# GREAT-WHU/DBA-Fusion

Hardware: AMD Instinct MI355X
Metric: DBA iterations/sec (25-KF, 96-edge, 512x512) [dba_update/s] (higher is better)
Workload: dtype f32 (BA, f64 reduced system) / f16 (correlation)

## Files before the change

dba-fusion_amd/csrc/ba_host.hip:

```cpp
#include <hip/hip_runtime.h>

#include <algorithm>
#include <atomic>
#include <cstdio>
#include <cstdlib>
#include <cstring>
#include <mutex>
#include <unordered_map>
#include <vector>

#include "ba_kernels.h"

#ifndef GRAM_F32_DEFAULT
#define GRAM_F32_DEFAULT true
#endif

namespace dba {

static thread_local char g_last_error[512] = "";

void set_last_error(const char *what, hipError_t e) {
  snprintf(g_last_error, sizeof(g_last_error), "%s -> %s", what, hipGetErrorString(e));
}

struct BaEnv {
  static int num(const char *name) { const char *e = getenv(name); return e ? atoi(e) : 0; }
  static bool is(const char *name, const char *prefix) { const char *e = getenv(name); return e && !strncmp(e, prefix, strlen(prefix)); }
  int deterministic = is("DBA_DETERMINISTIC", "1");
  int solve_check = is("DBA_SOLVE_CHECK", "1");
  int schur_form = is("DBA_SCHUR_KERNEL", "r") ? 1 : (is("DBA_SCHUR_KERNEL", "f") || is("DBA_SCHUR_KERNEL", "g")) ? 2 : 0;
  int lin_ppl = num("DBA_LINEARIZE_PPL");
  bool lin_no_mfma = is("DBA_LINEARIZE_MFMA", "0");
  int lin_ew = num("DBA_LIN_EW");
  bool h_full = is("DBA_H_FULL", "1");
  int schur_nch = num("DBA_SCHUR_NCH");
  int gram_threads = num("DBA_SCHUR_WAVES") == 4 ? 256 : 512;
  bool gram_f32 = getenv("DBA_SCHUR_MFMA") ? is("DBA_SCHUR_MFMA", "f3") : GRAM_F32_DEFAULT;
  bool fuse_update = !is("DBA_BA_FUSE_UPDATE", "0");
};
static const BaEnv &ba_env() { static const BaEnv env; return env; }

static std::atomic<int> g_schur_form{ba_env().schur_form};
static std::atomic<int> g_deterministic{ba_env().deterministic};
static std::atomic<int> g_solve_check{ba_env().solve_check};

__global__ __launch_bounds__(256) void ba_solve_check_kernel(const double *__restrict__ H, const double *__restrict__ b, int n, double lm,
                                                             double ep, float *__restrict__ dx, int *__restrict__ meta) {
  __shared__ double s_res[256], s_mag[256];
  __shared__ int s_bad;
  if (meta[1] != 0) return;
  double res = 0.0, mag = 0.0;
  for (int i = threadIdx.x; i < n; i += blockDim.x) {
    double acc = -b[i], m = fabs(b[i]);
    for (int j = 0; j < n; j++) {
      double h = H[(size_t)max(i, j) * n + min(i, j)];
      if (i == j) h = fma(lm, h, h) + ep;
      const double t = h * (double)dx[j];
      acc += t, m += fabs(t);
    }
    res = fmax(res, fabs(acc)), mag = fmax(mag, m);
  }
  s_res[threadIdx.x] = res, s_mag[threadIdx.x] = mag;
  __syncthreads();
  if (threadIdx.x == 0) {
    double r = 0.0, m = 0.0;
    for (int k = 0; k < (int)blockDim.x; k++) r = fmax(r, s_res[k]), m = fmax(m, s_mag[k]);
    s_bad = !(r <= 1e-5 * m) ? 1 : 0;
    if (s_bad) meta[1] = 1;
  }
  __syncthreads();
  if (s_bad)
    for (int i = threadIdx.x; i < n; i += blockDim.x) dx[i] = 0.f;
}

static bool schur_auto_frame_form(int N, int P) {
  const int frames = P + 1;
  const int rows_est = 1 + (N + frames - 1) / frames;
  return rows_est > 6;
}

static std::atomic<int> g_schur_generation{0};
static thread_local int t_schur_form = 0;

bool ba_schur_frame_form(int N, int P) {
  const int forced = g_schur_form.load(std::memory_order_relaxed);
  if (N + 1 > GRAM_LIST_CAP) return false;
  if (forced) return forced == 2;
  if (t_schur_form) return t_schur_form == 2;
  return schur_auto_frame_form(N, P);
}

// ... 64 lines not shown
    plan->T.meta = reinterpret_cast<int *>(base + L.meta);
    plan->T.kx = reinterpret_cast<int *>(base + L.kx);
    plan->T.frame_slot = reinterpret_cast<int *>(base + o_fslot);
    plan->T.eoff = reinterpret_cast<int *>(base + o_eoff);
    plan->T.elist = reinterpret_cast<int *>(base + o_elist);
    plan->T.elist_rank = reinterpret_cast<int *>(base + o_erank);
    plan->T.fpose = reinterpret_cast<int *>(base + o_fpose);
    plan->T.einfo = reinterpret_cast<int *>(base + o_einfo);
    plan->T.rowinfo = reinterpret_cast<int *>(base + o_rowinfo);
    plan->T.fhead = reinterpret_cast<int *>(base + o_fhead);
    plan->T.frow = reinterpret_cast<int *>(base + o_frow);
    plan->T.gkey = reinterpret_cast<int *>(base + o_gkey);
    plan->T.Mmax = Mmax;
    plan->T.B = B;
    plan->W.E = reinterpret_cast<float *>(base + L.E);
    plan->W.Q = reinterpret_cast<float *>(base + L.Q);
    plan->W.w = reinterpret_cast<float *>(base + L.w);
    plan->W.HpartE = reinterpret_cast<float *>(base + o_hparte);
    plan->W.Aedge = reinterpret_cast<double *>(base + o_aedge);
    plan->W.dx = reinterpret_cast<float *>(base + L.dx);
    plan->W.poses_tmp = reinterpret_cast<float *>(base + o_ptmp);
    plan->W.H = reinterpret_cast<double *>(base + L.H);
    plan->W.b = reinterpret_cast<double *>(base + L.b);
    plan->W.Lscratch = want_scratch ? reinterpret_cast<double *>(base + o_lscratch) : nullptr;
    plan->W.nparts = nparts;
    plan->W.ppl = ppl;
  }
  return DBA_OK;
}

static int ba_prepare_stage(const BaPlan &plan, const int64_t *ii, const int64_t *jj, int eta_rows, int check, bool judge_band,
                            hipStream_t stream) {
  const int N = plan.N, B = plan.B, P = plan.P;
  if (N > 0 && (!ii || !jj)) return DBA_ERR_ARG;
  const int want = std::max(std::max(N, B), P);
  const int threads = std::min(1024, std::max(64, (want + 63) / 64 * 64));
  const size_t scan_ints = std::max<size_t>(std::max(threads, P), N > threads ? 1024 : 0) + 32;
  const size_t lds = sizeof(int) * ((size_t)B + 2 * (size_t)plan.T.Mmax + 1 + scan_ints + plan.T.Mmax + 1);
  if (lds > 160 * 1024 || P > 16384) return DBA_ERR_UNSUPPORTED;
  if (lds > 64 * 1024) {
    DBA_HIP_CHECK(hipFuncSetAttribute(reinterpret_cast<const void *>(&ba_prepare_kernel),
                                      hipFuncAttributeMaxDynamicSharedMemorySize, 160 * 1024));
  }
  const int max_nt = judge_band ? ba_solve_wave_max_nt(6 * P) : 0;
  int *band_verdict = max_nt ? solver_verdict_slot(plan.T.meta) : nullptr;
  hipLaunchKernelGGL(ba_prepare_kernel, dim3(1), dim3(threads), lds, stream, ii, jj, N, B, plan.t0, plan.t1,
                     (int)scan_ints, ba_schur_frame_form(N, P) ? 1 : 0, check ? 1 : 0, eta_rows,
                     eta_rows > 1 ? ws_eta_status(plan.T.meta) : nullptr, plan.T, band_verdict, max_nt);
  DBA_LAUNCH_CHECK();
  return DBA_OK;
}

static int ba_linearize_stage(const BaPlan &plan, const BaProblem &g, const float *poses, const float *disps, float alpha,
                              int upd, float *poses_out, float *disps_w, hipStream_t stream) {
  if (!poses || !disps || !g.intrinsics || !g.disps_sens || !g.eta || g.eta_rows < 1) return DBA_ERR_ARG;
  if (g.eta_rows > 1 && g.eta_rows > plan.T.Mmax) return DBA_ERR_ARG;
  if (plan.N > 0 && (!g.targets || !g.weights || !g.jj)) return DBA_ERR_ARG;
#define LAUNCH_LIN(PPL, MF, EW)                                                                                          \
  hipLaunchKernelGGL((ba_linearize_kernel<PPL, MF, EW>), dim3(plan.nchunks * EW, plan.T.Mmax + 1), dim3(256), 0, stream, \
                     poses, disps, g.intrinsics, g.disps_sens, g.targets, g.weights, g.eta, g.eta_rows, g.jj,            \
                     g.frame_owned, plan.N, plan.HW, plan.wd, plan.t0, plan.P, alpha, upd, poses_out, disps_w, plan.T, plan.W)
  if (plan.W.ppl == 4) LAUNCH_LIN(4, false, 1);
  else if (plan.W.ppl == 2) LAUNCH_LIN(2, false, 1);
  else if (ba_env().lin_no_mfma) LAUNCH_LIN(1, false, 1);
  else {
    const int env_ew = ba_env().lin_ew;
    const long waves2 = (long)plan.nchunks * 2 * 4 * plan.T.Mmax;
    const bool one = env_ew ? env_ew == 1 : waves2 > 4096;
    if (one) LAUNCH_LIN(1, true, 1);
    else LAUNCH_LIN(1, true, 2);
  }
#undef LAUNCH_LIN
  DBA_LAUNCH_CHECK();
  return DBA_OK;
}

static int ba_reduce_stage(const BaPlan &plan, const int64_t *ii, const int64_t *jj, const uint8_t *frame_owned, int motion_only,
                           int lower, hipStream_t stream) {
  const int N = plan.N;
  const int ablocks = (N + 3) / 4;
  if (plan.P <= 0) return DBA_OK;
  if (ba_env().h_full) lower = 0;
  const bool fixed = g_deterministic.load(std::memory_order_relaxed) != 0;
  if (fixed) lower |= 2;
  if (!motion_only) {
    if (!ba_schur_frame_form(N, plan.P)) {
      hipLaunchKernelGGL(ba_schur_kernel, dim3(plan.P + N + ablocks, SCHUR_KP, SCHUR_CH), dim3(256), 0, stream, ii, jj,
                         frame_owned, N, plan.HW, plan.t0, plan.P, lower, plan.T, plan.W);
    } else {
      const int px = 1024;
      int nch = ba_env().schur_nch > 0 ? ba_env().schur_nch : (plan.HW + px - 1) / px;
      nch = std::max(1, std::min(nch, (plan.HW + 15) / 16));
      const dim3 grid((unsigned)(plan.T.Mmax * nch + ablocks));
      const int gram_threads = ba_env().gram_threads;
      const bool f32 = ba_env().gram_f32;
#define GRAM_LAUNCH(V, F)                                                                                     \
  hipLaunchKernelGGL((ba_schur_gram_kernel<V, F>), grid, dim3(gram_threads), 0, stream, ii, jj, frame_owned, \
                     N, plan.HW, plan.t0, plan.P, nch, lower, plan.T, plan.W)
      if (plan.HW % 4 == 0) { if (f32) GRAM_LAUNCH(true, true); else GRAM_LAUNCH(true, false); }
      else { if (f32) GRAM_LAUNCH(false, true); else GRAM_LAUNCH(false, false); }
#undef GRAM_LAUNCH
    }
    DBA_LAUNCH_CHECK();
  } else if (ablocks > 0) {
    hipLaunchKernelGGL(ba_assemble_kernel, dim3(ablocks), dim3(256), 0, stream, ii, jj, frame_owned, N, plan.t0, plan.P,
                       lower, plan.T, plan.W);
    DBA_LAUNCH_CHECK();
  }
  if (fixed) {
    const int n = 6 * plan.P;
    hipLaunchKernelGGL(ba_fixed_to_f64_kernel, dim3((n * n + n + 255) / 256), dim3(256), 0, stream, plan.W.H, plan.W.b, n);
    DBA_LAUNCH_CHECK();
  }
  return DBA_OK;
}

static int ba_symmetrize_launch(const BaPlan &plan, hipStream_t stream) {
  const int n = 6 * plan.P;
  if (n <= 0) return DBA_OK;
  hipLaunchKernelGGL(ba_symmetrize_kernel, dim3((n * n + 255) / 256), dim3(256), 0, stream, plan.W.H, n);
  DBA_LAUNCH_CHECK();
  return DBA_OK;
}

static int ba_solve_check_launch(const BaPlan &plan, float lm, float ep, hipStream_t stream) {
  if (plan.P <= 0) return DBA_OK;
  hipLaunchKernelGGL(ba_solve_check_kernel, dim3(1), dim3(256), 0, stream, plan.W.H, plan.W.b, 6 * plan.P, (double)lm, (double)ep,
                     plan.W.dx, plan.T.meta);
  DBA_LAUNCH_CHECK();
  return DBA_OK;
}

static int ba_solve_stage(const BaPlan &plan, float lm, float ep, const int *fpose, int hint, hipStream_t stream) {
  const int rc = launch_ba_solve(plan.W.H, plan.W.b, fpose, 6 * plan.P, (double)lm, (double)ep, plan.W.dx, plan.T.meta,
                                 plan.W.Lscratch, stream, nullptr, hint, (fpose && fpose == plan.T.fpose) ? plan.T.meta + 16 : nullptr);
  if (rc != DBA_OK) return rc;
  if (g_solve_check.load(std::memory_order_relaxed)) return ba_solve_check_launch(plan, lm, ep, stream);
  return DBA_OK;
}

static int ba_update_launch(const BaPlan &plan, float *poses, float *disps, const int64_t *jj, const uint8_t *frame_owned,
                            int update_poses, int update_disps, float *dz_out, float *dx_out, hipStream_t stream,
                            const float *poses_src = nullptr, float disp_floor = 0.f) {
  dim3 grid((plan.HW + 255) / 256, plan.T.Mmax + 1 + (disp_floor > 0.f ? plan.B : 0));
  hipLaunchKernelGGL(ba_update_kernel, grid, dim3(256), 0, stream, poses, poses_src, disps, jj, frame_owned, plan.HW, plan.t0,
                     plan.P, update_poses, update_disps, dz_out, dx_out, plan.T, plan.W, disp_floor);
  DBA_LAUNCH_CHECK();
  return DBA_OK;
}

int ba_run_loop(const BaPlan &plan, const BaProblem &g, float *poses, float *disps, const BaRun &run, hipStream_t stream) {
  const int *fpose = run.window_fpose ? run.window_fpose : plan.T.fpose;
  int rc;
  if (run.prepared != 1) {
    rc = ba_prepare_stage(plan, g.ii, g.jj, g.eta_rows, run.prepared == 2, run.window_fpose == nullptr, stream);
    if (rc != DBA_OK) return rc;
  }
  const bool fuse = ba_env().fuse_update;
  const float *pose_src = poses;
  bool pending = false;
  for (int itr = 0; itr < run.iterations; itr++) {
    float *pose_dst = plan.W.poses_tmp + (size_t)(itr & 1) * 7 * plan.B;
    const int upd = pending ? (run.motion_only ? 1 : 3) : 0;
    rc = ba_linearize_stage(plan, g, pose_src, disps, run.alpha, upd, pending ? pose_dst : nullptr, disps, stream);
    if (rc != DBA_OK) return rc;
    if (pending) pose_src = pose_dst;
    rc = ba_reduce_stage(plan, g.ii, g.jj, g.frame_owned, run.motion_only, 1, stream);
    if (rc != DBA_OK) return rc;
    if (run.exchange && run.exchange->fn && plan.P > 0) {
      const size_t n6 = (size_t)6 * plan.P;
      rc = run.exchange->fn(run.exchange->ctx, plan.W.H, (size_t)(plan.W.b - plan.W.H) + n6, stream);
      if (rc != DBA_OK) return rc;
    }
    rc = ba_solve_stage(plan, run.lm, run.ep, fpose, run.solver_hint, stream);
    if (rc != DBA_OK) return rc;
    const bool last = (itr == run.iterations - 1);
    if (fuse && !last) {
      pending = true;
      continue;
    }
    rc = ba_update_launch(plan, poses, disps, g.jj, g.frame_owned, 1, run.motion_only ? 0 : 1, last ? run.dz_out : nullptr,
                          last ? run.dx_out : nullptr, stream, pose_src == poses ? nullptr : pose_src,
                          last ? run.disp_floor : 0.f);
    if (rc != DBA_OK) return rc;
    pose_src = poses;
    pending = false;
  }
  return DBA_OK;
}

namespace {
struct BacoreStage {
  double *host = nullptr;
  size_t doubles = 0;
  unsigned *counter = nullptr;
  int seq = 0;
};
std::mutex g_stage_mu;
typedef std::unordered_map<const void *, BacoreStage> BacoreStageMap;
BacoreStageMap *stage_map_ptr() {
  static BacoreStageMap *m = new BacoreStageMap;
  return m;
}
#define stage_map() (*stage_map_ptr())
int *stage_flag(const BacoreStage &st) { return reinterpret_cast<int *>(st.host + st.doubles + 8); }
}

static int bacore_stage_for(const int *meta, size_t need, hipStream_t stream, BacoreStage **out) {
  std::lock_guard<std::mutex> lock(g_stage_mu);
  BacoreStage &st = stage_map()[meta];
  if (st.doubles < need) {
    if (st.host) {
      DBA_HIP_CHECK(hipStreamSynchronize(stream));
      (void)hipHostFree(st.host);
      st.host = nullptr, st.doubles = 0;
    }
    void *p = nullptr;
// ... 388 lines not shown
```

dba-fusion_amd/csrc/ba_kernels.h:

```cpp
#pragma once
#include "common.h"

namespace dba {

constexpr int HPE_STRIDE = 32;
#ifndef SCHUR_KP_CFG
#define SCHUR_KP_CFG 8
#endif
#ifndef SCHUR_CH_CFG
#define SCHUR_CH_CFG 2
#endif
constexpr int SCHUR_KP = SCHUR_KP_CFG;
constexpr int SCHUR_CH = SCHUR_CH_CFG;

struct BaTables {
  int *meta;
  int *kx;
  int *frame_slot;
  int *eoff;
  int *elist;
  int *elist_rank;
  int *fpose;
  int *einfo;
  int *rowinfo;
  int *fhead;
  int *frow;
  int *gkey;
  int Mmax, B;
};

struct BaBuffers {
  float *E;
  float *Q;
  float *w;
  float *HpartE;
  double *Aedge;
  double *H;
  double *b;
  float *dx;
  double *Lscratch;
  float *poses_tmp;
  int nparts;
  int ppl;
};

struct BaPlan {
  BaTables T;
  BaBuffers W;
  dba_ba_layout layout;
  size_t bytes;
  int P, N, B, HW, nchunks;
  int ht, wd, t0, t1;
};

int ba_plan(int N, int B, int ht, int wd, int t0, int t1, void *ws, size_t ws_bytes, BaPlan *plan);
#define DBA_PLAN_OR_RETURN(plan) \
  BaPlan plan;                   \
  if (const int plan_rc_ = ::dba::ba_plan(N, B, ht, wd, t0, t1, ws, ws_bytes, &plan)) return plan_rc_

constexpr int GKEY_MAGIC = 0x6b657935;
__global__ void ba_prepare_kernel(const int64_t *ii, const int64_t *jj, int N, int B, int t0, int t1, int scan_ints,
                                  int ftable, int check, int eta_rows, int *status, BaTables T, int *band_verdict, int max_nt);
bool ba_schur_frame_form(int N, int P);
template <int PPL, bool MF, int EW>
__global__ void ba_linearize_kernel(const float *poses, const float *disps, const float *intrinsics,
                                    const float *disps_sens, const float *targets, const float *weights,
                                    const float *eta, int eta_rows, const int64_t *jj,
                                    const uint8_t *frame_owned, int N, int HW, int wd, int t0, int P,
                                    float alpha, int upd, float *poses_out, float *disps_w, BaTables T, BaBuffers W);
__global__ void ba_assemble_kernel(const int64_t *ii, const int64_t *jj, const uint8_t *frame_owned, int N,
                                   int t0, int P, int lower, BaTables T, BaBuffers W);
__global__ void ba_schur_kernel(const int64_t *ii, const int64_t *jj, const uint8_t *frame_owned, int N, int HW,
                                int t0, int P, int lower, BaTables T, BaBuffers W);
__global__ void ba_symmetrize_kernel(double *H, int n);
struct ExportArg {
  double A[36];
};
__global__ void ba_export_kernel(const double *H, const double *b, int n, double *out, int gtsam, ExportArg arg, double stab,
                                 unsigned *counter, int *host_flag, int seq);
__global__ void ba_fixed_to_f64_kernel(double *H, double *b, int n);
constexpr int GRAM_LIST_CAP = 1024;
template <bool VEC, bool F32>
__global__ void ba_schur_gram_kernel(const int64_t *ii, const int64_t *jj, const uint8_t *frame_owned, int N, int HW,
                                     int t0, int P, int nch, int lower, BaTables T, BaBuffers W);
__global__ void ba_update_kernel(float *poses, const float *poses_src, float *disps, const int64_t *jj, const uint8_t *frame_owned,
                                 int HW, int t0, int P, int update_poses, int update_disps, float *dz_out,
                                 float *dx_out, BaTables T, BaBuffers W, float disp_floor);
__global__ void ba_copy_f32_kernel(const float *src, float *dst, int n);
__global__ void ba_gather_edges_kernel(const float2 *tgt_inac, const float2 *wgt_inac, const int64_t *ii_inac, const int64_t *jj_inac,
                                       const int64_t *sel, int n_sel, int n_inac, const float2 *tgt_act, const float2 *wgt_act,
                                       const int64_t *ii_act, const int64_t *jj_act, int HW, float *tgt_out, float *wgt_out,
                                       int64_t *ii_out, int64_t *jj_out);

struct BaProblem {
  const float *intrinsics, *disps_sens, *targets, *weights, *eta;
  int eta_rows;
  const int64_t *ii, *jj;
  const uint8_t *frame_owned;
};
struct BaExchange {
  int (*fn)(void *ctx, double *hb, size_t hb_len, hipStream_t stream);
  void *ctx;
};
struct BaRun {
  int iterations;
  float lm, ep, alpha;
  int motion_only;
  int prepared, solver_hint;
  float disp_floor;
  const int32_t *window_fpose;
  const BaExchange *exchange;
  float *dx_out, *dz_out;
};
int ba_run_loop(const BaPlan &plan, const BaProblem &g, float *poses, float *disps, const BaRun &run, hipStream_t stream);

int launch_ba_solve(const double *H, const double *b, const int *fpose, int n, double lm, double ep, float *dx, int *meta,
                    double *Lscratch, hipStream_t stream, long long *prof = nullptr, int hint = 0, int *splan = nullptr);
bool ba_solve_fits_lds(int n);
bool ba_solve_tile_supported(int n);
bool ba_solve_band_supported(int n);
int launch_ba_solve_band(const double *H, const double *b, const int *fpose, int n, double lm, double ep, float *dx,
                         int *meta, double *scratch, size_t scratch_doubles, bool big, hipStream_t stream,
// ... 16 lines not shown
```

dba-fusion_amd/csrc/ba_kernels.hip:

```cpp
#include "ba_kernels.h"
#include "ba_solve_admit.h"

#include <cstdio>
#include <cstring>

namespace dba {

__device__ __forceinline__ int wave_incl_scan(int v, int lane) {
#pragma unroll
  for (int off = 1; off < 64; off <<= 1) {
    const int o = __shfl_up(v, off, 64);
    if (lane >= off) v += o;
  }
  return v;
}

__global__ __launch_bounds__(1024) void ba_prepare_kernel(const int64_t *__restrict__ ii,
                                                          const int64_t *__restrict__ jj, int N, int B,
                                                          int t0, int t1, int scan_ints, int ftable, int check,
                                                          int eta_rows, int *__restrict__ status, BaTables T,
                                                          int *__restrict__ band_verdict, int max_nt) {
  extern __shared__ int sm[];
  int *flag = sm;
  int *cnt = sm + B;
  int *kxs = cnt + T.Mmax + 1;
  int *scan = kxs + T.Mmax;
  int *vcnt = scan + scan_ints;
  const int tid = threadIdx.x, nt = blockDim.x, lane = tid & 63, wave = tid >> 6, nw = nt >> 6;
  const int P = t1 - t0;
  const int my_i = (tid < N) ? (int)ii[tid] : -1, my_j = (tid < N) ? (int)jj[tid] : -1;
  auto src = [&](int n) { return (n == tid) ? my_i : (int)ii[n]; };
  auto dst = [&](int n) { return (n == tid) ? my_j : (int)jj[n]; };
  auto check_eta = [&](int nk) {
    if (tid == 0) {
      const bool bad = eta_rows > 1 && eta_rows != nk;
      T.gkey[7] = bad ? 1 : 0;
      if (bad && status) {
        status[1] = eta_rows, status[2] = nk;
        __hip_atomic_store(status, 1, __ATOMIC_RELEASE, __HIP_MEMORY_SCOPE_SYSTEM);
      }
    }
  };

  {
    const int *key = T.gkey;
    bool same = check && key[0] == GKEY_MAGIC && key[1] == N && key[2] == B && key[3] == t0 && key[4] == t1 &&
                key[5] == ftable && key[6] == T.Mmax;
    if (same) {
      for (int n = tid; n < N; n += nt) {
        const long long a = (long long)ii[n], b = (long long)jj[n];
        same = same && (long long)key[8 + n] == a && (long long)key[8 + N + n] == b;
      }
    }
    if (__syncthreads_and(same)) {
      check_eta(T.meta[0]);
      return;
    }
  }

  for (int f = tid; f < B; f += nt) flag[f] = 0;
  for (int m = tid; m <= T.Mmax; m += nt) cnt[m] = 0;
  __syncthreads();
  for (int p = tid; p < P; p += nt) {
    const int f = t0 + p;
    if (f >= 0 && f < B) flag[f] = 1;
  }
  for (int n = tid; n < N; n += nt) {
    const int f = src(n);
    if (f >= 0 && f < B) flag[f] = 1;
  }
  __syncthreads();

  const int per = (B + nt - 1) / nt;
  const int lo = min(tid * per, B), hi = min(lo + per, B);
  int c = 0;
// ... 129 lines not shown
        int rank = 0;
        const int qend = min(lim, n - base);
        for (int q = 0; q < qend; q++) rank += (sii[q] == f);
        T.elist_rank[n] += rank;
      }
    }
    __syncthreads();
    for (int n = tid; n < N; n += nt) {
      const int m = slot_of((int)ii[n]);
      const int pos = (m >= 0) ? cnt[m] + T.elist_rank[n] : -1;
      if (m >= 0) T.elist[pos] = n;
      emit_edge(n, m, pos, (int)jj[n]);
    }
  }
  for (int p = tid; p < P; p += nt) {
    const int m = slot_of(t0 + p);
    int *ri = T.rowinfo + 8 * p;
    ri[0] = m, ri[1] = p, ri[2] = (m >= 0) ? cnt[m] : 0, ri[3] = (m >= 0) ? cnt[m + 1] : 0, ri[4] = t0 + p;
  }
  __syncthreads();
  const int Mv = min(M, T.Mmax);
  int *minS = cnt;
  int *fps = scan;
  for (int m = tid; m < Mv; m += nt) {
    const int pp = kxs[m] - t0;
    minS[m] = (pp >= 0 && pp < P) ? pp : 0x7fffffff;
  }
  for (int pp = tid; pp < P; pp += nt) fps[pp] = pp;
  __syncthreads();
  for (int n = tid; n < N; n += nt) {
    const int m = slot_of(src(n)), tg = dst(n) - t0;
    if (m >= 0 && tg >= 0 && tg < P) atomicMin(&minS[m], tg);
  }
  __syncthreads();
  for (int n = tid; n < N; n += nt) {
    const int m = slot_of(src(n)), tg = dst(n) - t0;
    if (m >= 0 && tg >= 0 && tg < P) atomicMin(&fps[tg], minS[m]);
  }
  for (int m = tid; m < Mv; m += nt) {
    const int pp = kxs[m] - t0;
    if (pp >= 0 && pp < P) atomicMin(&fps[pp], minS[m]);
  }
  __syncthreads();
  for (int pp = tid; pp < P; pp += nt) T.fpose[pp] = fps[pp];
  if (band_verdict && wave == 0) {
    const int admitted = ba_solve_wave_admits(fps, 6 * P, lane, max_nt);
    if (lane == 0) __hip_atomic_store(band_verdict, admitted ? 1 : 2, __ATOMIC_RELAXED, __HIP_MEMORY_SCOPE_SYSTEM);
  }
  for (int n = tid; n < N; n += nt) T.gkey[8 + n] = (int)ii[n], T.gkey[8 + N + n] = (int)jj[n];
  if (tid == 0) {
    int *key = T.gkey;
    key[0] = GKEY_MAGIC, key[1] = N, key[2] = B, key[3] = t0, key[4] = t1, key[5] = ftable, key[6] = T.Mmax;
  }
}

__device__ void retract_pose(float *pose, const float *xi) {
  const float *tau = xi, *phi = xi + 3;
  const float th2 = phi[0] * phi[0] + phi[1] * phi[1] + phi[2] * phi[2];
  const float th4 = th2 * th2;
  const float th = sqrtf(th2);
  float imag, real;
  if (th2 < 1e-8f) {
    imag = 0.5f - (1.0f / 48.0f) * th2 + (1.0f / 3840.0f) * th4;
    real = 1.0f - (1.0f / 8.0f) * th2 + (1.0f / 384.0f) * th4;
  } else {
    imag = sinf(0.5f * th) / th;
    real = cosf(0.5f * th);
  }
  const float dq[4] = {imag * phi[0], imag * phi[1], imag * phi[2], real};
  float dt[3] = {tau[0], tau[1], tau[2]};
  if (th > 1e-4f) {
    const float a = (1.f - cosf(th)) / th2;
    const float b = (th - sinf(th)) / (th * th2);
    const float c1[3] = {phi[1] * tau[2] - phi[2] * tau[1], phi[2] * tau[0] - phi[0] * tau[2],
                         phi[0] * tau[1] - phi[1] * tau[0]};
    const float c2[3] = {phi[1] * c1[2] - phi[2] * c1[1], phi[2] * c1[0] - phi[0] * c1[2],
                         phi[0] * c1[1] - phi[1] * c1[0]};
#pragma unroll
    for (int c = 0; c < 3; c++) dt[c] += a * c1[c] + b * c2[c];
  }
  const float t[3] = {pose[0], pose[1], pose[2]};
  const float q[4] = {pose[3], pose[4], pose[5], pose[6]};
  float q1[4], t1[3];
  q1[0] = dq[3] * q[0] + dq[0] * q[3] + dq[1] * q[2] - dq[2] * q[1];
  q1[1] = dq[3] * q[1] + dq[1] * q[3] + dq[2] * q[0] - dq[0] * q[2];
  q1[2] = dq[3] * q[2] + dq[2] * q[3] + dq[0] * q[1] - dq[1] * q[0];
  q1[3] = dq[3] * q[3] - dq[0] * q[0] - dq[1] * q[1] - dq[2] * q[2];
  quat_rotate(dq, t, t1);
  pose[0] = t1[0] + dt[0];
  pose[1] = t1[1] + dt[1];
  pose[2] = t1[2] + dt[2];
  pose[3] = q1[0];
  pose[4] = q1[1];
  pose[5] = q1[2];
  pose[6] = q1[3];
}


__device__ __forceinline__ void load_pose(const float *__restrict__ poses, const float *__restrict__ dx, int f, int t0, int P,
                                          bool upd, float *out) {
#pragma unroll
  for (int c = 0; c < 7; c++) out[c] = poses[7 * f + c];
  const int p = f - t0;
  if (upd && p >= 0 && p < P) retract_pose(out, dx + 6 * p);
}

// ... 145 lines not shown
    s.y += v.y;
    s.z += v.z;
    s.w += v.w;
  }
  return (s.x + s.y) + (s.z + s.w);
}

__device__ __forceinline__ void wave_lds_fence() {
  __builtin_amdgcn_wave_barrier();
  __builtin_amdgcn_s_waitcnt(0xc07f);
  __builtin_amdgcn_wave_barrier();
}

template <int PPL, int A, int B_>
struct HjjLoop {
  __device__ __forceinline__ static void run(const PixelLin (&L)[PPL], float *acc) {
    float val = 0.f;
#pragma unroll
    for (int q = 0; q < PPL; q++)
      val += L[q].wu * L[q].Ju[A] * L[q].Ju[B_] + L[q].wv * L[q].Jv[A] * L[q].Jv[B_];
    reduce_deposit<A * (A + 1) / 2 + B_>(val, acc);
    if constexpr (B_ < A)
      HjjLoop<PPL, A, B_ + 1>::run(L, acc);
    else if constexpr (A < 5)
      HjjLoop<PPL, A + 1, 0>::run(L, acc);
  }
};

template <int PPL, int A>
struct VjLoop {
  __device__ __forceinline__ static void run(const PixelLin (&L)[PPL], float *acc) {
    float val = 0.f;
#pragma unroll
    for (int q = 0; q < PPL; q++) val += L[q].wu * L[q].ru * L[q].Ju[A] + L[q].wv * L[q].rv * L[q].Jv[A];
    reduce_deposit<21 + A>(val, acc);
    if constexpr (A < 5) VjLoop<PPL, A + 1>::run(L, acc);
  }
};

typedef float lin_f4 __attribute__((ext_vector_type(4)));
constexpr int MFS_T = 16;
constexpr int MFS_P = 20;
constexpr int MFS_VALS = 4 * 16 * MFS_P;
constexpr int MFS_WTS = 4 * 2 * MFS_P;
constexpr int MFS_FLOATS = (MFS_VALS + MFS_WTS) > (64 + 8 * 64) ? (MFS_VALS + MFS_WTS) : (64 + 8 * 64);

#ifdef LIN_PROF
__device__ unsigned long long g_lin_prof[16];
__device__ unsigned long long g_lin_span[2 * 8192];
#define LP(k) do { if (threadIdx.x == 0 && blockIdx.x == 3) { const unsigned long long t_ = wall_clock64(); atomicAdd(&g_lin_prof[k], t_ - lp_); lp_ = t_; } } while (0)
#else
#define LP(k) (void)0
#endif
template <int PPL, bool MF, int EW>
__global__ __launch_bounds__(256, (PPL == 1 ? (MF ? 4 : 2) : 1)) void ba_linearize_kernel(
    const float *__restrict__ poses, const float *__restrict__ disps, const float *__restrict__ intrinsics,
    const float *__restrict__ disps_sens, const float *__restrict__ targets,
    const float *__restrict__ weights, const float *__restrict__ eta, int eta_rows,
    const int64_t *__restrict__ jj, const uint8_t *__restrict__ frame_owned, int N, int HW, int wd,
    int t0, int P, float alpha, int upd_arg, float *__restrict__ poses_out, float *__restrict__ disps_w, BaTables T,
    BaBuffers W) {
  const int upd = T.gkey[7] ? 0 : upd_arg;
#ifdef LIN_PROF
  unsigned long long lp_ = wall_clock64();
  const unsigned long long lp_start_ = lp_;
#endif
  const int m = blockIdx.y;
  if (m == T.Mmax) {
    const int n6 = 6 * P;
    const size_t total = (size_t)n6 * n6;
    for (size_t i = (size_t)blockIdx.x * blockDim.x + threadIdx.x; i < total; i += (size_t)gridDim.x * blockDim.x)
      W.H[i] = 0.0;
    if (blockIdx.x == 0) {
      for (int i = threadIdx.x; i < n6; i += blockDim.x) W.b[i] = 0.0;
      if (upd && poses_out)
        for (int f = threadIdx.x; f < T.B; f += blockDim.x) {
          float pr[7];
          load_pose(poses, W.dx, f, t0, P, true, pr);
#pragma unroll
          for (int c = 0; c < 7; c++) poses_out[7 * f + c] = pr[c];
        }
    }
    return;
  }
  const int M = T.meta[0];
  if (m >= M) return;
  const int frame = T.kx[m];
  if (frame_owned && !frame_owned[frame]) return;

  const int lane = lane_id();
  const int wv = threadIdx.x >> 6, ew = wv % EW;
  const int wave_global = blockIdx.x * (4 / EW) + wv / EW;
  const int kbase = wave_global * (WAVE * PPL) + lane;
  const int nparts = W.nparts;

  float intr[4] = {intrinsics[0], intrinsics[1], intrinsics[2], intrinsics[3]};
  int kc[PPL];
  bool active[PPL];
  float u[PPL], v[PPL], disp[PPL];
#pragma unroll
  for (int q = 0; q < PPL; q++) {
    const int k = kbase + WAVE * q;
    active[q] = k < HW;
    kc[q] = active[q] ? k : 0;
    u[q] = (float)(kc[q] % wd);
    v[q] = (float)(kc[q] / wd);
    disp[q] = disps[(size_t)frame * HW + kc[q]];
    if ((upd & 2) && active[q])
      disp[q] = disp[q] + backsub_pixel(T, W, m, frame, kc[q], HW, t0, P);
  }
  if (upd & 2) {
    __syncthreads();
    if ((threadIdx.x >> 6) % EW == 0) {
#pragma unroll
      for (int q = 0; q < PPL; q++)
        if (active[q]) disps_w[(size_t)frame * HW + kc[q]] = disp[q];
    }
  }

  float Csum[PPL], wsum[PPL], Ei[PPL][6];
#pragma unroll
  for (int q = 0; q < PPL; q++) {
    Csum[q] = 0.f;
    wsum[q] = 0.f;
#pragma unroll
    for (int c = 0; c < 6; c++) Ei[q][c] = 0.f;
  }
  constexpr int EB = 16;
  __shared__ float s_pose[EB][12];
  __shared__ __attribute__((aligned(16))) float s_adj[EB][28];
  __shared__ int s_edge[EB][2];
  constexpr int RED_FLOATS = MF ? MFS_FLOATS : 64 * RED_PITCH;
  __shared__ __attribute__((aligned(16))) float s_red[4][RED_FLOATS];
  float *red_wave = s_red[wv];
  float *red_lane = red_wave + lane;
  const int e0 = T.eoff[m], e1 = T.eoff[m + 1];
  LP(0);
  for (int batch = e0; batch < e1; batch += EB) {
    const int cnt = min(EB, e1 - batch);
    __syncthreads();
    LP(1);
    if ((int)threadIdx.x < cnt) {
      const int2 ei = *reinterpret_cast<const int2 *>(T.einfo + 2 * (batch + threadIdx.x));
      const int n = ei.x, jx = ei.y;
      double t64[3], R64[9];
      edge_pose64(poses, W.dx, frame, jx, t0, P, upd != 0, t64, R64);
      s_edge[threadIdx.x][0] = n;
      s_edge[threadIdx.x][1] = jx;
#pragma unroll
      for (int c = 0; c < 3; c++) s_pose[threadIdx.x][c] = (float)t64[c];
#pragma unroll
      for (int c = 0; c < 9; c++) s_pose[threadIdx.x][3 + c] = (float)R64[c];
      double *Aw = (blockIdx.x == 0) ? W.Aedge + (size_t)n * 36 : nullptr;
      float *As = s_adj[threadIdx.x];
#pragma unroll
      for (int k = 0; k < 3; k++) {
#pragma unroll
        for (int c = 0; c < 3; c++) {
          const double rkc = -R64[3 * k + c];
          const int k1 = (k + 1) % 3, k2 = (k + 2) % 3;
          const double x = t64[k2] * R64[3 * k1 + c] - t64[k1] * R64[3 * k2 + c];
          As[6 * k + c] = (float)rkc, As[6 * k + 3 + c] = (float)x, As[18 + 3 * k + c] = (float)rkc;
          if (Aw) Aw[6 * k + c] = rkc, Aw[6 * k + 3 + c] = x, Aw[6 * (3 + k) + c] = 0.0, Aw[6 * (3 + k) + 3 + c] = rkc;
        }
      }
    }
    __syncthreads();
    LP(2);
    float nx_t[PPL][2], nx_w[PPL][2];
    {
      const int n = s_edge[min(ew, cnt - 1)][0];
#pragma unroll
      for (int q = 0; q < PPL; q++) {
        const size_t tb = (size_t)n * 2 * HW + kc[q];
        nx_t[q][0] = targets[tb];
        nx_t[q][1] = targets[tb + HW];
        nx_w[q][0] = weights[tb];
        nx_w[q][1] = weights[tb + HW];
      }
    }
    for (int i = ew; i < cnt; i += EW) {
      const int n = s_edge[i][0];
      const int jx = s_edge[i][1];
      float tij[3];
      Rot3 R;
#pragma unroll
      for (int c = 0; c < 3; c++) tij[c] = s_pose[i][c];
#pragma unroll
      for (int c = 0; c < 9; c++) R.r[c] = s_pose[i][3 + c];
      float cu_t[PPL][2], cu_w[PPL][2];
#pragma unroll
      for (int q = 0; q < PPL; q++) {
        cu_t[q][0] = nx_t[q][0]; cu_t[q][1] = nx_t[q][1];
        cu_w[q][0] = nx_w[q][0]; cu_w[q][1] = nx_w[q][1];
      }
      if (i + EW < cnt) {
// ... 147 lines not shown
    W.w[(size_t)m * HW + k] = w;
    const int p = frame - t0;
    if (p >= 0 && p < P) {
      float *Er = W.E + ((size_t)p * 6) * HW + k;
#pragma unroll
      for (int c = 0; c < 6; c++) Er[(size_t)c * HW] = Ei[q][c];
    }
  }
  LP(5);
#ifdef LIN_PROF
  if ((threadIdx.x & 63) == 0) {
    const int slot = ((blockIdx.y * gridDim.x + blockIdx.x) * 4 + (threadIdx.x >> 6)) & 8191;
    g_lin_span[2 * slot] = lp_start_;
    g_lin_span[2 * slot + 1] = wall_clock64();
  }
#endif
}

#ifdef LIN_PROF
extern "C" void dba_lin_prof_dump() {
  unsigned long long h[16];
  (void)hipDeviceSynchronize();
  (void)hipMemcpyFromSymbol(h, HIP_SYMBOL(g_lin_prof), sizeof(h));
  static unsigned long long sp[2 * 8192];
  (void)hipMemcpyFromSymbol(sp, HIP_SYMBOL(g_lin_span), sizeof(sp));
  unsigned long long lo = ~0ull, hi = 0, sum = 0, cnt = 0, maxlife = 0, laststart = 0;
  for (int i = 0; i < 8192; i++)
    if (sp[2 * i]) {
      lo = sp[2 * i] < lo ? sp[2 * i] : lo, hi = sp[2 * i + 1] > hi ? sp[2 * i + 1] : hi;
      laststart = sp[2 * i] > laststart ? sp[2 * i] : laststart;
      const unsigned long long life = sp[2 * i + 1] - sp[2 * i];
      sum += life, cnt++, maxlife = life > maxlife ? life : maxlife;
    }
  fprintf(stderr, "LIN_PROF (10 ns ticks, wave 0 of slice-block 3, summed over frames): prologue %llu, sync %llu, resolve %llu, edges %llu, tail-of-loop %llu, epilogue %llu | last launch: %llu waves, first start -> last end %llu ticks, last start at +%llu, mean life %.1f, longest %llu\n",
          h[0], h[1], h[2], h[3], h[4], h[5], cnt, hi - lo, laststart - lo, cnt ? (double)sum / cnt : 0.0, maxlife);
  {
    fprintf(stderr, "LIN_PROF residency (t in ticks: alive / started):");
    for (int d = 0; d <= 10; d++) {
      const unsigned long long t = lo + (hi - lo) * d / 10;
      int alive = 0, started = 0;
      for (int i = 0; i < 8192; i++)
        if (sp[2 * i]) started += sp[2 * i] <= t, alive += (sp[2 * i] <= t && sp[2 * i + 1] > t);
      fprintf(stderr, " %llu: %d / %d;", t - lo, alive, started);
    }
    fprintf(stderr, "\n");
  }
  memset(h, 0, sizeof(h));
  memset(sp, 0, sizeof(sp));
  (void)hipMemcpyToSymbol(HIP_SYMBOL(g_lin_span), sp, sizeof(sp));
  (void)hipMemcpyToSymbol(HIP_SYMBOL(g_lin_prof), h, sizeof(h));
}
#endif

template __global__ void ba_linearize_kernel<1, true, 2>(const float *, const float *, const float *, const float *,
                                                const float *, const float *, const float *, int, const int64_t *,
                                                const uint8_t *, int, int, int, int, int, float, int, float *, float *,
                                                BaTables, BaBuffers);
template __global__ void ba_linearize_kernel<1, true, 1>(const float *, const float *, const float *, const float *,
                                                const float *, const float *, const float *, int, const int64_t *,
                                                const uint8_t *, int, int, int, int, int, float, int, float *, float *,
                                                BaTables, BaBuffers);
template __global__ void ba_linearize_kernel<1, false, 1>(const float *, const float *, const float *, const float *,
                                                const float *, const float *, const float *, int, const int64_t *,
                                                const uint8_t *, int, int, int, int, int, float, int, float *, float *,
                                                BaTables, BaBuffers);
template __global__ void ba_linearize_kernel<2, false, 1>(const float *, const float *, const float *, const float *,
                                                const float *, const float *, const float *, int, const int64_t *,
                                                const uint8_t *, int, int, int, int, int, float, int, float *, float *,
                                                BaTables, BaBuffers);
template __global__ void ba_linearize_kernel<4, false, 1>(const float *, const float *, const float *, const float *,
                                                const float *, const float *, const float *, int, const int64_t *,
                                                const uint8_t *, int, int, int, int, int, float, int, float *, float *,
                                                BaTables, BaBuffers);

__device__ __forceinline__ void atomic_add_f64(double *p, double v) {
  __hip_atomic_fetch_add(p, v, __ATOMIC_RELAXED, __HIP_MEMORY_SCOPE_AGENT);
}

constexpr double ACC_FIX_SCALE = 1073741824.0;
__device__ __forceinline__ void acc_add(double *p, double v, bool fixed) {
  if (fixed)
    atomicAdd(reinterpret_cast<unsigned long long *>(p), (unsigned long long)__double2ll_rn(v * ACC_FIX_SCALE));
  else
    atomic_add_f64(p, v);
}

__device__ __forceinline__ void h_add_pair(const BaBuffers &W, int n6, int hr, int hc, double s, bool lower, bool fixed) {
  if (lower) {
    if (hr == hc) acc_add(&W.H[(size_t)hr * n6 + hc], 2.0 * s, fixed);
    else acc_add(&W.H[(size_t)max(hr, hc) * n6 + min(hr, hc)], s, fixed);
  } else {
    acc_add(&W.H[(size_t)hr * n6 + hc], s, fixed);
    acc_add(&W.H[(size_t)hc * n6 + hr], s, fixed);
  }
}


__device__ __forceinline__ void ba_assemble_block(int block, const int64_t *__restrict__ ii,
                                                  const int64_t *__restrict__ jj,
                                                  const uint8_t *__restrict__ frame_owned, int N, int t0, int P,
                                                  int hflags, const BaTables &T, const BaBuffers &W) {
  const bool lower = (hflags & 1) != 0, fixed = (hflags & 2) != 0;
  const int tid = threadIdx.x;
  const int n6 = 6 * P;
  const int edge_blocks = (N + 3) / 4;
  if (block < edge_blocks) {
    const int n = 4 * block + (tid >> 6);
    const int l = tid & 63;
    if (n >= N) return;
    const int src = (int)ii[n];
    if (frame_owned && !frame_owned[src]) return;
    int ta = 0;
    while ((ta + 1) * (ta + 2) / 2 <= min(l, 20)) ta++;
    const int tb = min(l, 20) - ta * (ta + 1) / 2;
    const int ja = min(l, 35) / 6, jb = min(l, 35) % 6;
    const int va = (l >= 21 && l < 27) ? l - 21 : 0;
    double Ajb[6], Atb[6], Ata[6], Ava[6];
    {
      const double *A = W.Aedge + (size_t)n * 36;
#pragma unroll
      for (int k = 0; k < 6; k++) Ajb[k] = A[6 * k + jb], Atb[k] = A[6 * k + tb], Ata[k] = A[6 * k + ta], Ava[k] = A[6 * k + va];
    }
    double s = 0.0;
    if (l < 27) {
      const float *hp = W.HpartE + (size_t)n * W.nparts * HPE_STRIDE + l;
      int part = 0;
// ... 578 lines not shown
```

Before: 3958.

## Fold prepare stage into first linearize launch to drop a kernel

When the plan is freshly prepared (prepared==2) and conditions are simple, the separate single-block prepare kernel is skipped. Its work runs in an extra grid row of the first linearize launch, and each linearize block rebuilds its frame list and edge list itself from ii/jj using shared-memory bitmasks and ballots. This removes one serialized launch and the dependency on prepare's tables for iteration zero. In exchange, every block repeats the edge scan, LDS staging is reused for the prepare body, and there are new template instantiations.

```diff
diff --git a/dba-fusion_amd/csrc/ba_host.hip b/dba-fusion_amd/csrc/ba_host.hip
--- a/dba-fusion_amd/csrc/ba_host.hip
+++ b/dba-fusion_amd/csrc/ba_host.hip
@@ -23,6 +23,7 @@
   snprintf(g_last_error, sizeof(g_last_error), "%s -> %s", what, hipGetErrorString(e));
 }
 
+constexpr bool STAGE0_FOLD_DEFAULT = true;
 struct BaEnv {
   static int num(const char *name) { const char *e = getenv(name); return e ? atoi(e) : 0; }
   static bool is(const char *name, const char *prefix) { const char *e = getenv(name); return e && !strncmp(e, prefix, strlen(prefix)); }
@@ -37,6 +38,7 @@
   int gram_threads = num("DBA_SCHUR_WAVES") == 4 ? 256 : 512;
   bool gram_f32 = getenv("DBA_SCHUR_MFMA") ? is("DBA_SCHUR_MFMA", "f3") : GRAM_F32_DEFAULT;
   bool fuse_update = !is("DBA_BA_FUSE_UPDATE", "0");
+  bool stage0_fold = getenv("DBA_BA_STAGE0") ? is("DBA_BA_STAGE0", "fold") : STAGE0_FOLD_DEFAULT;
 };
 static const BaEnv &ba_env() { static const BaEnv env; return env; }
 
@@ -207,16 +209,20 @@
 }
 
 static int ba_linearize_stage(const BaPlan &plan, const BaProblem &g, const float *poses, const float *disps, float alpha,
-                              int upd, float *poses_out, float *disps_w, hipStream_t stream) {
+                              int upd, float *poses_out, float *disps_w, hipStream_t stream, const BaStage0 *s0 = nullptr) {
   if (!poses || !disps || !g.intrinsics || !g.disps_sens || !g.eta || g.eta_rows < 1) return DBA_ERR_ARG;
   if (g.eta_rows > 1 && g.eta_rows > plan.T.Mmax) return DBA_ERR_ARG;
   if (plan.N > 0 && (!g.targets || !g.weights || !g.jj)) return DBA_ERR_ARG;
-#define LAUNCH_LIN(PPL, MF, EW)                                                                                          \
-  hipLaunchKernelGGL((ba_linearize_kernel<PPL, MF, EW>), dim3(plan.nchunks * EW, plan.T.Mmax + 1), dim3(256), 0, stream, \
-                     poses, disps, g.intrinsics, g.disps_sens, g.targets, g.weights, g.eta, g.eta_rows, g.jj,            \
-                     g.frame_owned, plan.N, plan.HW, plan.wd, plan.t0, plan.P, alpha, upd, poses_out, disps_w, plan.T, plan.W)
-  if (plan.W.ppl == 4) LAUNCH_LIN(4, false, 1);
-  else if (plan.W.ppl == 2) LAUNCH_LIN(2, false, 1);
+  if (s0 && (upd != 0 || plan.W.ppl != 1)) return DBA_ERR_ARG;
+  const BaStage0 none = {nullptr, 0, 0, nullptr, nullptr, 0};
+#define LAUNCH_LIN_TF(PPL, MF, EW, TF)                                                                                        \
+  hipLaunchKernelGGL((ba_linearize_kernel<PPL, MF, EW, TF>), dim3(plan.nchunks * EW, plan.T.Mmax + (TF ? 2 : 1)), dim3(256), 0, \
+                     stream, poses, disps, g.intrinsics, g.disps_sens, g.targets, g.weights, g.eta, g.eta_rows, g.jj,         \
+                     g.frame_owned, plan.N, plan.HW, plan.wd, plan.t0, plan.P, alpha, upd, poses_out, disps_w, plan.T, plan.W, \
+                     TF ? *s0 : none)
+#define LAUNCH_LIN(PPL, MF, EW) do { if (s0) LAUNCH_LIN_TF(PPL, MF, EW, true); else LAUNCH_LIN_TF(PPL, MF, EW, false); } while (0)
+  if (plan.W.ppl == 4) LAUNCH_LIN_TF(4, false, 1, false);
+  else if (plan.W.ppl == 2) LAUNCH_LIN_TF(2, false, 1, false);
   else if (ba_env().lin_no_mfma) LAUNCH_LIN(1, false, 1);
   else {
     const int env_ew = ba_env().lin_ew;
@@ -226,6 +232,7 @@
     else LAUNCH_LIN(1, true, 2);
   }
 #undef LAUNCH_LIN
+#undef LAUNCH_LIN_TF
   DBA_LAUNCH_CHECK();
   return DBA_OK;
 }
@@ -304,10 +311,22 @@
   return DBA_OK;
 }
 
+static bool ba_stage0_folds(const BaPlan &plan, const BaProblem &g, const BaRun &run) {
+  return ba_env().stage0_fold && run.prepared == 2 && run.iterations > 0 && !g.frame_owned && !run.exchange && !run.window_fpose &&
+         plan.W.ppl == 1 && plan.N <= FOLD_MAX_N && plan.B <= FOLD_MAX_B && (plan.N == 0 || (g.ii && g.jj));
+}
+
 int ba_run_loop(const BaPlan &plan, const BaProblem &g, float *poses, float *disps, const BaRun &run, hipStream_t stream) {
   const int *fpose = run.window_fpose ? run.window_fpose : plan.T.fpose;
   int rc;
-  if (run.prepared != 1) {
+  const bool fold = ba_stage0_folds(plan, g, run);
+  BaStage0 s0 = {nullptr, 0, 0, nullptr, nullptr, 0};
+  if (fold) {
+    const int max_nt = ba_solve_wave_max_nt(6 * plan.P);
+    s0.ii = g.ii, s0.t1 = plan.t1, s0.ftable = ba_schur_frame_form(plan.N, plan.P) ? 1 : 0;
+    s0.status = g.eta_rows > 1 ? ws_eta_status(plan.T.meta) : nullptr;
+    s0.band_verdict = max_nt ? solver_verdict_slot(plan.T.meta) : nullptr, s0.max_nt = max_nt;
+  } else if (run.prepared != 1) {
     rc = ba_prepare_stage(plan, g.ii, g.jj, g.eta_rows, run.prepared == 2, run.window_fpose == nullptr, stream);
     if (rc != DBA_OK) return rc;
   }
@@ -317,7 +336,8 @@
   for (int itr = 0; itr < run.iterations; itr++) {
     float *pose_dst = plan.W.poses_tmp + (size_t)(itr & 1) * 7 * plan.B;
     const int upd = pending ? (run.motion_only ? 1 : 3) : 0;
-    rc = ba_linearize_stage(plan, g, pose_src, disps, run.alpha, upd, pending ? pose_dst : nullptr, disps, stream);
+    rc = ba_linearize_stage(plan, g, pose_src, disps, run.alpha, upd, pending ? pose_dst : nullptr, disps, stream,
+                            (fold && itr == 0) ? &s0 : nullptr);
     if (rc != DBA_OK) return rc;
     if (pending) pose_src = pose_dst;
     rc = ba_reduce_stage(plan, g.ii, g.jj, g.frame_owned, run.motion_only, 1, stream);
diff --git a/dba-fusion_amd/csrc/ba_kernels.h b/dba-fusion_amd/csrc/ba_kernels.h
--- a/dba-fusion_amd/csrc/ba_kernels.h
+++ b/dba-fusion_amd/csrc/ba_kernels.h
@@ -62,12 +62,21 @@
 __global__ void ba_prepare_kernel(const int64_t *ii, const int64_t *jj, int N, int B, int t0, int t1, int scan_ints,
                                   int ftable, int check, int eta_rows, int *status, BaTables T, int *band_verdict, int max_nt);
 bool ba_schur_frame_form(int N, int P);
-template <int PPL, bool MF, int EW>
+struct BaStage0 {
+  const int64_t *ii;
+  int t1, ftable;
+  int *status, *band_verdict;
+  int max_nt;
+};
+constexpr int FOLD_MAX_N = 256, FOLD_MAX_B = 512;
+constexpr int FOLD_SCAN_INTS = FOLD_MAX_B + 32;
+template <int PPL, bool MF, int EW, bool TF>
 __global__ void ba_linearize_kernel(const float *poses, const float *disps, const float *intrinsics,
                                     const float *disps_sens, const float *targets, const float *weights,
                                     const float *eta, int eta_rows, const int64_t *jj,
                                     const uint8_t *frame_owned, int N, int HW, int wd, int t0, int P,
-                                    float alpha, int upd, float *poses_out, float *disps_w, BaTables T, BaBuffers W);
+                                    float alpha, int upd, float *poses_out, float *disps_w, BaTables T, BaBuffers W,
+                                    BaStage0 S0);
 __global__ void ba_assemble_kernel(const int64_t *ii, const int64_t *jj, const uint8_t *frame_owned, int N,
                                    int t0, int P, int lower, BaTables T, BaBuffers W);
 __global__ void ba_schur_kernel(const int64_t *ii, const int64_t *jj, const uint8_t *frame_owned, int N, int HW,
diff --git a/dba-fusion_amd/csrc/ba_kernels.hip b/dba-fusion_amd/csrc/ba_kernels.hip
--- a/dba-fusion_amd/csrc/ba_kernels.hip
+++ b/dba-fusion_amd/csrc/ba_kernels.hip
@@ -15,12 +15,9 @@
   return v;
 }
 
-__global__ __launch_bounds__(1024) void ba_prepare_kernel(const int64_t *__restrict__ ii,
-                                                          const int64_t *__restrict__ jj, int N, int B,
-                                                          int t0, int t1, int scan_ints, int ftable, int check,
-                                                          int eta_rows, int *__restrict__ status, BaTables T,
-                                                          int *__restrict__ band_verdict, int max_nt) {
-  extern __shared__ int sm[];
+__device__ void ba_prepare_body(int *sm, const int64_t *__restrict__ ii, const int64_t *__restrict__ jj, int N, int B, int t0,
+                                int t1, int scan_ints, int ftable, int check, int eta_rows, int *__restrict__ status,
+                                const BaTables &T, int *__restrict__ band_verdict, int max_nt) {
   int *flag = sm;
   int *cnt = sm + B;
   int *kxs = cnt + T.Mmax + 1;
@@ -256,6 +253,15 @@
     int *key = T.gkey;
     key[0] = GKEY_MAGIC, key[1] = N, key[2] = B, key[3] = t0, key[4] = t1, key[5] = ftable, key[6] = T.Mmax;
   }
+}
+
+__global__ __launch_bounds__(1024) void ba_prepare_kernel(const int64_t *__restrict__ ii,
+                                                          const int64_t *__restrict__ jj, int N, int B,
+                                                          int t0, int t1, int scan_ints, int ftable, int check,
+                                                          int eta_rows, int *__restrict__ status, BaTables T,
+                                                          int *__restrict__ band_verdict, int max_nt) {
+  extern __shared__ int sm[];
+  ba_prepare_body(sm, ii, jj, N, B, t0, t1, scan_ints, ftable, check, eta_rows, status, T, band_verdict, max_nt);
 }
 
 __device__ void retract_pose(float *pose, const float *xi) {
@@ -507,20 +513,35 @@
 #else
 #define LP(k) (void)0
 #endif
-template <int PPL, bool MF, int EW>
+template <int PPL, bool MF, int EW, bool TF>
 __global__ __launch_bounds__(256, (PPL == 1 ? (MF ? 4 : 2) : 1)) void ba_linearize_kernel(
     const float *__restrict__ poses, const float *__restrict__ disps, const float *__restrict__ intrinsics,
     const float *__restrict__ disps_sens, const float *__restrict__ targets,
     const float *__restrict__ weights, const float *__restrict__ eta, int eta_rows,
     const int64_t *__restrict__ jj, const uint8_t *__restrict__ frame_owned, int N, int HW, int wd,
     int t0, int P, float alpha, int upd_arg, float *__restrict__ poses_out, float *__restrict__ disps_w, BaTables T,
-    BaBuffers W) {
-  const int upd = T.gkey[7] ? 0 : upd_arg;
+    BaBuffers W, BaStage0 S0) {
+  const int upd = TF ? 0 : (T.gkey[7] ? 0 : upd_arg);
 #ifdef LIN_PROF
   unsigned long long lp_ = wall_clock64();
   const unsigned long long lp_start_ = lp_;
 #endif
+  constexpr int EB = 16;
+  __shared__ float s_pose[EB][12];
+  __shared__ __attribute__((aligned(16))) float s_adj[EB][28];
+  __shared__ int s_edge[EB][2];
+  constexpr int RED_FLOATS = MF ? MFS_FLOATS : 64 * RED_PITCH;
+  __shared__ __attribute__((aligned(16))) float s_red[4][RED_FLOATS];
   const int m = blockIdx.y;
+  if constexpr (TF) {
+    if (m == T.Mmax + 1) {
+      static_assert(!TF || 4 * FOLD_MAX_B + 2 + FOLD_SCAN_INTS <= 4 * RED_FLOATS, "stage 0 does not fit the staging tiles");
+      if (blockIdx.x == 0)
+        ba_prepare_body(reinterpret_cast<int *>(&s_red[0][0]), S0.ii, jj, N, T.B, t0, S0.t1, FOLD_SCAN_INTS, S0.ftable, 1, eta_rows,
+                        S0.status, T, S0.band_verdict, S0.max_nt);
+      return;
+    }
+  }
   if (m == T.Mmax) {
     const int n6 = 6 * P;
     const size_t total = (size_t)n6 * n6;
@@ -538,10 +559,53 @@
     }
     return;
   }
-  const int M = T.meta[0];
-  if (m >= M) return;
-  const int frame = T.kx[m];
-  if (frame_owned && !frame_owned[frame]) return;
+  int frame, e0 = 0, e1 = 0;
+  __shared__ int2 s_out[TF ? FOLD_MAX_N : 1];
+  if constexpr (TF) {
+    __shared__ unsigned s_fmask[FOLD_MAX_B / 32];
+    __shared__ int s_wcnt[4];
+    const int tid = threadIdx.x;
+    const int my_i = (tid < N) ? (int)S0.ii[tid] : -1, my_j = (tid < N) ? (int)jj[tid] : -1;
+    if (tid < FOLD_MAX_B / 32) {
+      const int lo = min(max(t0 - 32 * tid, 0), 32), hi = min(max(S0.t1 - 32 * tid, 0), 32);
+      const unsigned below_hi = (hi >= 32) ? ~0u : ((1u << hi) - 1u), below_lo = (lo >= 32) ? ~0u : ((1u << lo) - 1u);
+      s_fmask[tid] = below_hi & ~below_lo;
+    }
+    __syncthreads();
+    if (my_i >= 0 && my_i < T.B) atomicOr(&s_fmask[my_i >> 5], 1u << (my_i & 31));
+    __syncthreads();
+    int M = 0, word = 0, skip = 0;
+    unsigned bits = 0;
+    bool found = false;
+#pragma unroll
+    for (int w = 0; w < FOLD_MAX_B / 32; w++) {
+      const unsigned b = s_fmask[w];
+      const int c = __popc(b);
+      if (!found && m < M + c) found = true, word = w, bits = b, skip = m - M;
+      M += c;
+    }
+    if (m >= min(M, T.Mmax)) return;
+    for (int r = 0; r < skip; r++) bits &= bits - 1;
+    frame = 32 * word + __ffs(bits) - 1;
+    if (frame_owned && !frame_owned[frame]) return;
+    const bool mine = my_i == frame;
+    const unsigned long long bal = __ballot(mine);
+    if ((tid & 63) == 0) s_wcnt[tid >> 6] = __popcll(bal);
+    __syncthreads();
+    int before = 0;
+#pragma unroll
+    for (int w = 0; w < 4; w++) {
+      const int c = s_wcnt[w];
+      before += (w < (tid >> 6)) ? c : 0;
+      e1 += c;
+    }
+    if (mine) s_out[before + __popcll(bal & ((1ull << (tid & 63)) - 1ull))] = make_int2(tid, my_j);
+  } else {
+    const int M = T.meta[0];
+    if (m >= M) return;
+    frame = T.kx[m];
+    if (frame_owned && !frame_owned[frame]) return;
+  }
 
   const int lane = lane_id();
   const int wv = threadIdx.x >> 6, ew = wv % EW;
@@ -581,22 +645,16 @@
 #pragma unroll
     for (int c = 0; c < 6; c++) Ei[q][c] = 0.f;
   }
-  constexpr int EB = 16;
-  __shared__ float s_pose[EB][12];
-  __shared__ __attribute__((aligned(16))) float s_adj[EB][28];
-  __shared__ int s_edge[EB][2];
-  constexpr int RED_FLOATS = MF ? MFS_FLOATS : 64 * RED_PITCH;
-  __shared__ __attribute__((aligned(16))) float s_red[4][RED_FLOATS];
   float *red_wave = s_red[wv];
   float *red_lane = red_wave + lane;
-  const int e0 = T.eoff[m], e1 = T.eoff[m + 1];
+  if constexpr (!TF) e0 = T.eoff[m], e1 = T.eoff[m + 1];
   LP(0);
   for (int batch = e0; batch < e1; batch += EB) {
     const int cnt = min(EB, e1 - batch);
     __syncthreads();
     LP(1);
     if ((int)threadIdx.x < cnt) {
-      const int2 ei = *reinterpret_cast<const int2 *>(T.einfo + 2 * (batch + threadIdx.x));
+      const int2 ei = TF ? s_out[batch + threadIdx.x] : *reinterpret_cast<const int2 *>(T.einfo + 2 * (batch + threadIdx.x));
       const int n = ei.x, jx = ei.y;
       double t64[3], R64[9];
       edge_pose64(poses, W.dx, frame, jx, t0, P, upd != 0, t64, R64);
@@ -850,26 +908,20 @@
 }
 #endif
 
-template __global__ void ba_linearize_kernel<1, true, 2>(const float *, const float *, const float *, const float *,
-                                                const float *, const float *, const float *, int, const int64_t *,
-                                                const uint8_t *, int, int, int, int, int, float, int, float *, float *,
-                                                BaTables, BaBuffers);
-template __global__ void ba_linearize_kernel<1, true, 1>(const float *, const float *, const float *, const float *,
-                                                const float *, const float *, const float *, int, const int64_t *,
-                                                const uint8_t *, int, int, int, int, int, float, int, float *, float *,
-                                                BaTables, BaBuffers);
-template __global__ void ba_linearize_kernel<1, false, 1>(const float *, const float *, const float *, const float *,
-                                                const float *, const float *, const float *, int, const int64_t *,
-                                                const uint8_t *, int, int, int, int, int, float, int, float *, float *,
-                                                BaTables, BaBuffers);
-template __global__ void ba_linearize_kernel<2, false, 1>(const float *, const float *, const float *, const float *,
-                                                const float *, const float *, const float *, int, const int64_t *,
-                                                const uint8_t *, int, int, int, int, int, float, int, float *, float *,
-                                                BaTables, BaBuffers);
-template __global__ void ba_linearize_kernel<4, false, 1>(const float *, const float *, const float *, const float *,
-                                                const float *, const float *, const float *, int, const int64_t *,
-                                                const uint8_t *, int, int, int, int, int, float, int, float *, float *,
-                                                BaTables, BaBuffers);
+#define LIN_INST(PPL, MF, EW, TF)                                                                                          \
+  template __global__ void ba_linearize_kernel<PPL, MF, EW, TF>(const float *, const float *, const float *, const float *,  \
+                                                                const float *, const float *, const float *, int,            \
+                                                                const int64_t *, const uint8_t *, int, int, int, int, int,   \
+                                                                float, int, float *, float *, BaTables, BaBuffers, BaStage0)
+LIN_INST(1, true, 2, false);
+LIN_INST(1, true, 1, false);
+LIN_INST(1, false, 1, false);
+LIN_INST(2, false, 1, false);
+LIN_INST(4, false, 1, false);
+LIN_INST(1, true, 2, true);
+LIN_INST(1, true, 1, true);
+LIN_INST(1, false, 1, true);
+#undef LIN_INST
 
 __device__ __forceinline__ void atomic_add_f64(double *p, double v) {
   __hip_atomic_fetch_add(p, v, __ATOMIC_RELAXED, __HIP_MEMORY_SCOPE_AGENT);
```

Measured after the change: 4037 (median of 6 runs). +2.0%, better.
